# software-mansion/smelter

Measured on AMD Instinct MI355X. Metric: composited frames/sec, 8x1080p->1 4K scene, higher is better.
Workload: dtype u8 (f32 colour conversion: the WGSL sequence value for value; Lanczos on f16-pair MFMA with f32 accumulate, f16 resampler intermediate); 1 GPU; configs[2]: 8x1080p YUV420 inputs tiled -> 3840x2160 YUV420, Tiles + Rescaler(border_radius 24) + text label per tile, GpuOptimized (linear-light Lanczos3 + blend); inputs=8, layouts=33, prime_frames=4804, input_ring=12, frames_in_flight=2, parallelism=single GPU

## Files before the change

### smelter_amd/csrc/smr_fused_compose.h

```cpp
#pragma once

#include <type_traits>

#include "smr_convert_dev.h"
#include "smr_layout_dev.h"

namespace {

#ifdef SMR_EMU
#define B_KEEP_IN_LOOP(x) do { } while (0)
#else
#define B_KEEP_IN_LOOP(x) asm volatile("" : "+v"(x))
#endif

__device__ __forceinline__ u32 b_off(int row, u32 pitch, int col_bytes) { return (u32)__umul24((u32)row, pitch) + (u32)col_bytes; }

constexpr int B_TILE_W = 128, B_TILE_H = 16;
constexpr int B_MAX_LAYOUTS = 48;
constexpr int B_MAX_MASKS = 96;
static_assert(sizeof(DevLayout) % 16 == 0 && sizeof(DevMask) % 16 == 0, "LDS copies move 16 B words");

#ifndef SMR_COMPOSE_MIN_WAVES
#define SMR_COMPOSE_MIN_WAVES 6
#endif
constexpr int B_MIN_WAVES = SMR_COMPOSE_MIN_WAVES;
constexpr int B_BAND_ROWS = SMR_COMPOSE_BAND_ROWS;
static_assert(B_TILE_H % B_BAND_ROWS == 0 && B_BAND_ROWS >= 2, "a band fits the LDS pixel state");

inline u32 compose_predict(const PackedLayouts &p, int tiles_x, int tiles_y, std::vector<u32> &bitmap) {
    const int tiles = tiles_x * tiles_y, words = (tiles + 31) / 32;
    bitmap.assign((size_t)words, 0u);
    auto mark = [&](float x0, float y0, float x1, float y1) {
        int tx0 = (int)floorf(x0 / (float)B_TILE_W), tx1 = (int)floorf(x1 / (float)B_TILE_W);
        int ty0 = (int)floorf(y0 / (float)B_TILE_H), ty1 = (int)floorf(y1 / (float)B_TILE_H);
        tx0 = tx0 < 0 ? 0 : tx0; ty0 = ty0 < 0 ? 0 : ty0;
        tx1 = tx1 >= tiles_x ? tiles_x - 1 : tx1; ty1 = ty1 >= tiles_y ? tiles_y - 1 : ty1;
        for (int ty = ty0; ty <= ty1; ty++)
            for (int tx = tx0; tx <= tx1; tx++) {
                const int t = ty * tiles_x + tx;
                bitmap[t >> 5] |= 1u << (t & 31);
            }
    };
    auto corners = [&](float left, float top, float w, float h, float c, const DevLayout &L) {
        if (!(c > 0.0f)) return;
        const float bx0 = (float)L.bx0, by0 = (float)L.by0, bx1 = (float)L.bx1 - 1.0f, by1 = (float)L.by1 - 1.0f;
        const float xs[2][2] = {{left, left + c}, {left + w - c, left + w}}, ys[2][2] = {{top, top + c}, {top + h - c, top + h}};
        for (int a = 0; a < 2; a++)
            for (int b = 0; b < 2; b++) {
                const float x0 = fmaxf(xs[a][0], bx0), x1 = fminf(xs[a][1], bx1), y0 = fmaxf(ys[b][0], by0), y1 = fminf(ys[b][1], by1);
                if (x0 <= x1 && y0 <= y1) mark(x0, y0, x1, y1);
            }
    };
    for (int i = 0; i < p.n; i++) {
        const DevLayout &L = p.host_layouts[i];
        if (L.bx1 <= L.bx0 || L.by1 <= L.by0) continue;
        const bool solid_capable = (L.flags & DL_UNROTATED) && (L.type == 0 ? L.src_kind == 2 : (L.flags & DL_COLOR_OPAQUE) != 0);
        if (!solid_capable) {
            mark((float)L.bx0, (float)L.by0, (float)L.bx1 - 1.0f, (float)L.by1 - 1.0f);
            continue;
        }
        corners(L.left, L.top, L.width, L.height, L.corner, L);
        for (u32 m = 0; m < L.masks_len; m++) {
            const DevMask &K = p.host_masks[L.masks_off + m];
            corners(K.left, K.top, K.width, K.height, K.corner, L);
            if (K.left > L.left || K.top > L.top || K.left + K.width < L.left + L.width || K.top + K.height < L.top + L.height)
                mark((float)L.bx0, (float)L.by0, (float)L.bx1 - 1.0f, (float)L.by1 - 1.0f);
        }
        if (L.inset != 0.5f) {
            const float d = ceilf(L.inset);
            const float x0 = (float)L.bx0, y0 = (float)L.by0, x1 = (float)L.bx1 - 1.0f, y1 = (float)L.by1 - 1.0f;
            mark(x0, y0, x1, fminf(y0 + d, y1)); mark(x0, fmaxf(y1 - d, y0), x1, y1);
            mark(x0, y0, fminf(x0 + d, x1), y1); mark(fmaxf(x1 - d, x0), y0, x1, y1);
        }
    }
    u32 nf = 0;
    for (int w = 0; w < words; w++) nf += (u32)__builtin_popcount(bitmap[w]);
    return nf;
}

__device__ __forceinline__ void classify_layouts(u32 *s_touch, u32 *s_solid, int *s_start, const DevLayout *__restrict__ layouts,
                                                 const DevMask *__restrict__ masks, int n, int x0, int y0, int x1, int y1, int tid,
                                                 int nthreads) {
    if (tid < MAX_LAYOUT_WORDS) { s_touch[tid] = 0; s_solid[tid] = 0; }
    if (tid == 0) *s_start = -1;
    __syncthreads();
    const float cx0 = (float)x0 + 0.5f, cx1 = (float)x1 - 0.5f, cy0 = (float)y0 + 0.5f, cy1 = (float)y1 - 0.5f;
    for (int i = tid; i < n; i += nthreads) {
        const DevLayout &L = layouts[i];
        if (!(L.bx0 < x1 && L.bx1 > x0 && L.by0 < y1 && L.by1 > y0)) continue;
        atomicOr(&s_touch[i >> 5], 1u << (i & 31));
        if (!layout_solid_box(L, masks, cx0, cy0, cx1, cy1)) continue;
        atomicOr(&s_solid[i >> 5], 1u << (i & 31));
        if (layout_base_opaque(L)) atomicMax(s_start, i);
    }
    __syncthreads();
}

__device__ __forceinline__ void tile_needs(const u32 *s_touch, int start, int *s_general, const DevLayout *__restrict__ layouts, int n, int tid,
                                           int nthreads) {
    for (int i = tid; i < n; i += nthreads) {
        if (!((s_touch[i >> 5] >> (i & 31)) & 1u) || i < start) continue;
        const DevLayout &L = layouts[i];
        const bool copy_layer = i == start && (L.type != 0 || (L.flags & DL_ALIGNED));
        const bool sample_layer = i == start && L.type == 0 && !(L.flags & DL_ALIGNED);
        if (sample_layer) atomicOr(s_general, 2);
        else if (!copy_layer) atomicOr(s_general, 1);
        if (!(layout_base_opaque(L) && (L.flags & DL_UNROTATED))) atomicOr(s_general, 4);
    }
}

enum { TC_CLEAR = 0, TC_COLOUR = 1, TC_TEXTURE = 2, TC_FULL = 3, TC_SKIP = 4, TC_SAMPLED = 5, TC_SELECT = 6 };
struct alignas(16) TileClass {
    const u8 *base;
    u32 pitch_or_px;
    u32 kind;
};
struct TileFull {
    u32 tile;
    int start;
    u32 general;
    u32 band;
    u32 touch[MAX_LAYOUT_WORDS];
};
constexpr int B_AREA_BANDS = 4, B_EDGE_BANDS = B_TILE_H / B_BAND_ROWS;
static_assert(B_TILE_H / B_AREA_BANDS <= B_BAND_ROWS && B_EDGE_BANDS <= B_AREA_BANDS, "a band fits the workgroup's pixel state");
constexpr int B_LIST_COUNTERS = 64;
struct TileList {
    u32 count[B_LIST_COUNTERS];
    TileFull e[1];
};
constexpr u32 B_CLASS_NONE = 0xffu;
constexpr int B_CLASSIFY_TILES = 16;
__global__ __launch_bounds__(64 * B_CLASSIFY_TILES) void k_classify_tiles(const DevLayout *__restrict__ layouts, const DevMask *__restrict__ masks, int n,
                                                                          int W, int H, int tiles_x, int tiles, unsigned long long direct_layers,
                                                                          TileClass *__restrict__ tc, u8 *__restrict__ direct, TileList *__restrict__ full,
                                                                          int allow_select, int counter) {
    __shared__ u32 s_touch_w[B_CLASSIFY_TILES][MAX_LAYOUT_WORDS], s_solid_w[B_CLASSIFY_TILES][MAX_LAYOUT_WORDS];
    __shared__ int s_start_w[B_CLASSIFY_TILES], s_general_w[B_CLASSIFY_TILES], s_slot_w[B_CLASSIFY_TILES];
    __shared__ TileClass s_class_w[B_CLASSIFY_TILES];
    __shared__ u32 s_direct_w[B_CLASSIFY_TILES];
    const int wave = threadIdx.x >> 6, tid = threadIdx.x & 63;
    const bool live = (int)blockIdx.x * B_CLASSIFY_TILES + wave < tiles;
    const int tile = min((int)blockIdx.x * B_CLASSIFY_TILES + wave, tiles - 1);
    u32 *s_touch = s_touch_w[wave], *s_solid = s_solid_w[wave];
    int &s_start = s_start_w[wave], &s_general = s_general_w[wave], &s_slot = s_slot_w[wave];
    const int tile_y = tile / tiles_x;
    const int tx0 = (tile - tile_y * tiles_x) * B_TILE_W, ty0 = tile_y * B_TILE_H;
    if (tid == 0) s_general = 0;
    classify_layouts(s_touch, s_solid, &s_start, layouts, masks, n, tx0, ty0, min(tx0 + B_TILE_W, W), min(ty0 + B_TILE_H, H), tid, 64);
    const int start = s_start;
    tile_needs(s_touch, start, &s_general, layouts, n, tid, 64);
    __syncthreads();
    if (tid == 0) {
        TileClass c;
        c.base = nullptr; c.pitch_or_px = 0u; c.kind = TC_FULL;
        u32 d = B_CLASS_NONE;
        if ((s_general & 3) == 1 && allow_select) {
            const int x1 = min(tx0 + B_TILE_W, W), y1 = min(ty0 + B_TILE_H, H);
            u32 ids = 0xffffffffu;
            int cnt = 0;
            bool ok = true;
            for (int wi = (n + 31) / 32 - 1; ok && wi >= 0; wi--) {
                u32 bits = s_touch[wi];
                while (ok && bits) {
                    const int b = 31 - __clz(bits);
                    bits &= ~(1u << b);
                    const int i = wi * 32 + b;
                    if (i < start) continue;
                    const DevLayout &L = layouts[i];
                    const int ax0 = max(L.bx0, tx0), ay0 = max(L.by0, ty0), ax1 = min(L.bx1, x1), ay1 = min(L.by1, y1);
                    ok = cnt < 4 && i < 255 && layout_base_opaque(L) && (L.type != 0 || (L.flags & DL_ALIGNED)) &&
                         layout_solid_box(L, masks, (float)ax0 + 0.5f, (float)ay0 + 0.5f, (float)ax1 - 0.5f, (float)ay1 - 0.5f);
                    if (ok) {
                        ids = (ids & ~(0xffu << (8 * cnt))) | ((u32)i << (8 * cnt));
                        cnt++;
                    }
                }
            }
            if (ok && cnt > 0) {
                c.kind = TC_SELECT;
                c.pitch_or_px = ids;
            }
        } else if ((s_general & 3) == 2 && start >= 0) {
            c.kind = TC_SAMPLED;
            c.pitch_or_px = (u32)start;
        } else if ((s_general & 3) == 0) {
            if (start < 0) {
                c.kind = TC_CLEAR;
            } else if (layouts[start].type != 0) {
                c.kind = TC_COLOUR;
                c.pitch_or_px = layouts[start].solid_px;
            } else {
                const DevLayout &L = layouts[start];
                c.kind = TC_TEXTURE;
                c.base = L.src.ptr + (ptrdiff_t)(ty0 - L.iy) * (ptrdiff_t)L.src.pitch + (ptrdiff_t)(tx0 - L.ix) * 4;
                c.pitch_or_px = (u32)L.src.pitch;
                if (start < 64 && ((direct_layers >> start) & 1ull) && tx0 + B_TILE_W <= W && ty0 + B_TILE_H <= H) {
                    c.kind = TC_SKIP;
                    d = (u32)start;
                }
            }
        }
        s_slot = (live && c.kind == TC_FULL) ? ((s_general & 4) ? B_AREA_BANDS : B_EDGE_BANDS) : 0;
        s_class_w[wave] = c;
        s_direct_w[wave] = d;
    }
    __syncthreads();
    if (threadIdx.x == 0) {
        int want = 0;
        for (int w = 0; w < B_CLASSIFY_TILES; w++) want += s_slot_w[w];
        const u32 base = want ? atomicAdd(&full->count[counter], (u32)want) : 0u;
        int at = 0;
        for (int w = 0; w < B_CLASSIFY_TILES; w++) {
            const int mine = s_slot_w[w] ? (int)base + at : -1;
            at += s_slot_w[w];
            s_slot_w[w] = mine;
        }
    }
    __syncthreads();
    const int bands = (s_general & 4) ? B_AREA_BANDS : B_EDGE_BANDS;
    if (tid == 0 && live) {
        TileClass c = s_class_w[wave];
        if (c.kind == TC_FULL) { c.pitch_or_px = (u32)s_slot; c.base = (const u8 *)(uintptr_t)bands; }
        tc[tile] = c;
        direct[tile] = (u8)s_direct_w[wave];
    }
    if (s_slot >= 0) {
        const int rows = B_TILE_H / bands;
        for (int j = 0; j < bands; j++) {
            TileFull &E = full->e[s_slot + j];
            if (tid < MAX_LAYOUT_WORDS) E.touch[tid] = tid < ((n + 31) >> 5) ? s_touch[tid] : 0u;
            if (tid == 0) { E.tile = (u32)tile; E.start = start; E.general = (u32)s_general; E.band = (u32)(j * rows) | ((u32)rows << 8); }
        }
    }
}

template <typename T>
__device__ __forceinline__ T load_uniform(const T *p) {
    static_assert(sizeof(T) % 4 == 0, "dword records only");
    T out;
#pragma unroll
    for (int i = 0; i < (int)(sizeof(T) / 4); i++) {
        u32 w;
        __builtin_memcpy(&w, (const char *)p + 4 * i, 4);
        w = __builtin_amdgcn_readfirstlane(w);
        __builtin_memcpy((char *)&out + 4 * i, &w, 4);
    }
    return out;
}

__device__ __forceinline__ float4 decode_texel(u32 raw, int srgb, const float *__restrict__ dec) {
    const u32 r = raw & 0xff, g = (raw >> 8) & 0xff, b = (raw >> 16) & 0xff, a = raw >> 24;
    float4 o;
    if (srgb) { o.x = dec[r]; o.y = dec[g]; o.z = dec[b]; }
    else { o.x = (float)r / 255.0f; o.y = (float)g / 255.0f; o.z = (float)b / 255.0f; }
    o.w = div_cr((float)a, 255.0f, 1.0f / 255.0f);
    return o;
}

__device__ __forceinline__ u32 aligned_texel(const DevLayout &L, int px, int py) {
    return g_ld_u32(L.src.ptr + b_off(clampi(py - L.iy, 0, L.tex_h - 1), L.src.pitch, clampi(px - L.ix, 0, L.tex_w - 1) * 4));
}

__device__ __forceinline__ u32 compose_px(u32 a, const DevLayout &L, const DevMask *__restrict__ masks, int px, int py, bool is_base,
                                          u32 raw_pre, int srgb, const float *__restrict__ dec, const float *__restrict__ thr) {
    float fx, fy, lx, ly;
    if (!layout_covers(L, px, py, fx, fy, lx, ly)) return a;
    const bool solid = is_base || layout_solid_box(L, masks, fx, fy, fx, fy);
    if (L.type != 0) {
        if (solid && (L.flags & DL_COLOR_OPAQUE)) return L.solid_px;
        const float4 frag = solid ? make_float4(L.color[0], L.color[1], L.color[2], L.color[3])
                                  : layout_fragment(L, masks, fx, fy, lx, ly, make_float4(0.f, 0.f, 0.f, 0.f));
        return blend_store(a, frag, srgb, dec, thr);
    }
    const bool aligned = (L.flags & DL_ALIGNED) && L.src_kind != 0;
    u32 raw = 0u;
    float4 sample;
    if (aligned) {
        raw = raw_pre;
        sample = decode_texel(raw, srgb, dec);
    } else {
        sample = layout_texture_sample(L, px, py, lx, ly, srgb, dec);
    }
    const float4 frag = solid ? sample : layout_fragment(L, masks, fx, fy, lx, ly, sample);
    if (aligned && (raw >> 24) == 255u && frag.x == sample.x && frag.y == sample.y && frag.z == sample.z && frag.w == sample.w) return raw;
    return blend_store(a, frag, srgb, dec, thr);
}

__device__ __forceinline__ void yuv_block_repair(const u32 (&acc)[8], u32 &yrow0, u32 &yrow1, u32 &u2, u32 &v2) {
    u32 px[8];
    float r[8], g[8], b[8];
#pragma unroll
    for (int k = 0; k < 8; k++) {
        px[k] = acc[k];
        B_KEEP_IN_LOOP(px[k]);
        r[k] = unorm_of_byte(px[k] & 0xffu);
        g[k] = unorm_of_byte((px[k] >> 8) & 0xffu);
        b[k] = unorm_of_byte((px[k] >> 16) & 0xffu);
    }
#pragma unroll
    for (int k = 0; k < 8; k++) {
        bool f;
        (void)yuvfast::convert<0>((float)(px[k] & 0xffu), (float)((px[k] >> 8) & 0xffu), (float)((px[k] >> 16) & 0xffu), &f);
        const u32 exact = yuv_byte(r[k], g[k], b[k], 0), sh = 8u * (u32)(k & 3);
        u32 &row = k < 4 ? yrow0 : yrow1;
        row = f ? ((row & ~(0xffu << sh)) | (exact << sh)) : row;
    }
#pragma unroll
    for (int j = 0; j < 2; j++) {
        const int a = 2 * j, c = 4 + 2 * j;
        float sum[3];
#pragma unroll
        for (int ch = 0; ch < 3; ch++)
            sum[ch] = ((float)((px[a] >> (8 * ch)) & 0xffu) + (float)((px[a + 1] >> (8 * ch)) & 0xffu)) +
                      ((float)((px[c] >> (8 * ch)) & 0xffu) + (float)((px[c + 1] >> (8 * ch)) & 0xffu));
        bool f1, f2;
        (void)yuvfast::convert<1>(sum[0], sum[1], sum[2], &f1);
        (void)yuvfast::convert<2>(sum[0], sum[1], sum[2], &f2);
        const float mr = ((r[a] + r[a + 1]) + (r[c] + r[c + 1])) * 0.25f, mg = ((g[a] + g[a + 1]) + (g[c] + g[c + 1])) * 0.25f,
                    mb = ((b[a] + b[a + 1]) + (b[c] + b[c + 1])) * 0.25f;
        const u32 eu = yuv_byte(mr, mg, mb, 1), ev = yuv_byte(mr, mg, mb, 2), sh = 8u * (u32)j;
        u2 = f1 ? ((u2 & ~(0xffu << sh)) | (eu << sh)) : u2;
        v2 = f2 ? ((v2 & ~(0xffu << sh)) | (ev << sh)) : v2;
    }
}


__device__ __forceinline__ void yuv_block_repair_422(const u32 (&acc)[8], u32 &yrow0, u32 &yrow1, u32 &uv0, u32 &uv1) {
    u32 px[8];
    float r[8], g[8], b[8];
#pragma unroll
    for (int k = 0; k < 8; k++) {
        px[k] = acc[k];
        B_KEEP_IN_LOOP(px[k]);
        r[k] = unorm_of_byte(px[k] & 0xffu);
        g[k] = unorm_of_byte((px[k] >> 8) & 0xffu);
        b[k] = unorm_of_byte((px[k] >> 16) & 0xffu);
    }
#pragma unroll
    for (int k = 0; k < 8; k++) {
        bool f;
        (void)yuvfast::convert<0>((float)(px[k] & 0xffu), (float)((px[k] >> 8) & 0xffu), (float)((px[k] >> 16) & 0xffu), &f);
        const u32 exact = yuv_byte(r[k], g[k], b[k], 0), sh = 8u * (u32)(k & 3);
        u32 &row = k < 4 ? yrow0 : yrow1;
        row = f ? ((row & ~(0xffu << sh)) | (exact << sh)) : row;
    }
#pragma unroll
    for (int q = 0; q < 4; q++) {
        const int a = 4 * (q >> 1) + 2 * (q & 1);
        float sum[3];
#pragma unroll
        for (int ch = 0; ch < 3; ch++) sum[ch] = (float)((px[a] >> (8 * ch)) & 0xffu) + (float)((px[a + 1] >> (8 * ch)) & 0xffu);
        bool f1, f2;
        (void)yuvfast::convert422<1>(sum[0], sum[1], sum[2], &f1);
        (void)yuvfast::convert422<2>(sum[0], sum[1], sum[2], &f2);
        const float mr = r[a] * 0.5f + r[a + 1] * 0.5f, mg = g[a] * 0.5f + g[a + 1] * 0.5f, mb = b[a] * 0.5f + b[a + 1] * 0.5f;
        const u32 eu = yuv_byte(mr, mg, mb, 1), ev = yuv_byte(mr, mg, mb, 2), su = 8u * (u32)(q & 1), sv = su + 16u;
        u32 &uv = q < 2 ? uv0 : uv1;
        uv = f1 ? ((uv & ~(0xffu << su)) | (eu << su)) : uv;
        uv = f2 ? ((uv & ~(0xffu << sv)) | (ev << sv)) : uv;
    }
}

template <int NV>
__device__ __forceinline__ u32 packed422_texel(u32 y4, u32 uv, int j) {
    const u32 ya = (y4 >> (16 * j)) & 0xffu, yb = (y4 >> (16 * j + 8)) & 0xffu, u = (uv >> (8 * j)) & 0xffu, v = (uv >> (16 + 8 * j)) & 0xffu;
    return NV == 3 ? u | (ya << 8) | (v << 16) | (yb << 24) : ya | (u << 8) | (yb << 16) | (v << 24);
}

__device__ __forceinline__ bool plane_pair_aligned_422(const SurfView &p) { return ((((uintptr_t)p.ptr) | p.pitch) & 15u) == 0; }

template <int NV>
__device__ __forceinline__ void store_packed422_block(const u32 (&acc)[8], int px0, int py0, int W, const SurfView &p, bool pair) {
    float cr[8], cg[8], cb[8];
#pragma unroll
    for (int k = 0; k < 8; k++) {
        cr[k] = (float)(acc[k] & 0xffu);
        cg[k] = (float)((acc[k] >> 8) & 0xffu);
        cb[k] = (float)((acc[k] >> 16) & 0xffu);
    }
    u32 yrow0 = 0, yrow1 = 0, uv0 = 0, uv1 = 0;
    bool flagged = false;
#pragma unroll
    for (int k = 0; k < 4; k++) {
        bool f0, f1;
        yrow0 |= yuvfast::convert<0>(cr[k], cg[k], cb[k], &f0) << (8 * k);
        yrow1 |= yuvfast::convert<0>(cr[4 + k], cg[4 + k], cb[4 + k], &f1) << (8 * k);
        flagged |= f0 | f1;
    }
#pragma unroll
    for (int q = 0; q < 4; q++) {
        const int a = 4 * (q >> 1) + 2 * (q & 1);
        const float sr = cr[a] + cr[a + 1], sg = cg[a] + cg[a + 1], sb = cb[a] + cb[a + 1];
        bool f1, f2;
        const u32 c = (yuvfast::convert422<1>(sr, sg, sb, &f1) << (8 * (q & 1))) | (yuvfast::convert422<2>(sr, sg, sb, &f2) << (16 + 8 * (q & 1)));
        if (q < 2) uv0 |= c; else uv1 |= c;
        flagged |= f1 | f2;
    }
    if (flagged) {
        YUV_SLOW_PATH_STAYS_A_BRANCH();
        yuv_block_repair_422(acc, yrow0, yrow1, uv0, uv1);
    }
    const u32 t00 = packed422_texel<NV>(yrow0, uv0, 0), t01 = packed422_texel<NV>(yrow0, uv0, 1);
    const u32 t10 = packed422_texel<NV>(yrow1, uv1, 0), t11 = packed422_texel<NV>(yrow1, uv1, 1);
    if (pair) {
        const bool odd = (px0 & 4) != 0;
        const u32 n0 = (u32)dev_mov_dpp_quad_swap((int)(odd ? t00 : t10)), n1 = (u32)dev_mov_dpp_quad_swap((int)(odd ? t01 : t11));
        g_st_u32x4(p.ptr + b_off(py0 + (odd ? 1 : 0), p.pitch, (px0 & ~7) * 2), odd ? make_uint4(n0, n1, t10, t11) : make_uint4(t00, t01, n0, n1));
        return;
    }
    u8 *o = p.ptr + b_off(py0, p.pitch, px0 * 2);
    if (px0 + 3 >= W) {
        g_st_u32(o, t00);
        g_st_u32(o + p.pitch, t10);
    } else {
        g_st_u32x2(o, t00, t01);
        g_st_u32x2(o + p.pitch, t10, t11);
    }
}

template <int NV>
__device__ __forceinline__ bool planes_pair_aligned(const SurfView &yp, const SurfView &up, const SurfView &vp) {
#if defined(SMR_EMU) && !defined(SMR_EMU_WAVE_EXCHANGE)
    return false;
#else
    if (NV >= 3) return plane_pair_aligned_422(yp);
    if (NV == 2) return false;
    bool ok = ((((uintptr_t)yp.ptr) | yp.pitch) & 7u) == 0;
    if (NV == 0) ok = ok && ((((uintptr_t)up.ptr) | up.pitch | ((uintptr_t)vp.ptr) | vp.pitch) & 3u) == 0;
    return ok;
#endif
}

template <int NV>
__device__ __forceinline__ void store_yuv_block(const u32 (&acc)[8], int px0, int py0, int W, const SurfView &yp, const SurfView &up, const SurfView &vp,
                                                bool pair = false) {
    if (NV >= 3) {
        store_packed422_block<NV>(acc, px0, py0, W, yp, pair);
        return;
    }
    const bool half = px0 + 3 >= W;
    if (NV == 2) {
        u8 *o = yp.ptr + b_off(py0, yp.pitch, px0 * 4);
        if (half) {
            *(uint2 *)o = make_uint2(acc[0], acc[1]);
            *(uint2 *)(o + yp.pitch) = make_uint2(acc[4], acc[5]);
        } else {
            *(uint4 *)o = make_uint4(acc[0], acc[1], acc[2], acc[3]);
            *(uint4 *)(o + yp.pitch) = make_uint4(acc[4], acc[5], acc[6], acc[7]);
        }
        return;
    }
    float cr[8], cg[8], cb[8];
#pragma unroll
    for (int k = 0; k < 8; k++) {
        cr[k] = (float)(acc[k] & 0xffu);
        cg[k] = (float)((acc[k] >> 8) & 0xffu);
        cb[k] = (float)((acc[k] >> 16) & 0xffu);
    }
    u32 yrow0 = 0, yrow1 = 0, u2 = 0, v2 = 0;
    bool flagged = false;
#pragma unroll
    for (int k = 0; k < 4; k++) {
        bool f0, f1;
        yrow0 |= yuvfast::convert<0>(cr[k], cg[k], cb[k], &f0) << (8 * k);
        yrow1 |= yuvfast::convert<0>(cr[4 + k], cg[4 + k], cb[4 + k], &f1) << (8 * k);
        flagged |= f0 | f1;
    }
#pragma unroll
    for (int j = 0; j < 2; j++) {
        const int a = 2 * j, b = 2 * j + 1, c = 4 + 2 * j, d = 4 + 2 * j + 1;
        const float sr = (cr[a] + cr[b]) + (cr[c] + cr[d]), sg = (cg[a] + cg[b]) + (cg[c] + cg[d]), sb = (cb[a] + cb[b]) + (cb[c] + cb[d]);
        bool f1, f2;
        u2 |= yuvfast::convert<1>(sr, sg, sb, &f1) << (8 * j);
        v2 |= yuvfast::convert<2>(sr, sg, sb, &f2) << (8 * j);
        flagged |= f1 | f2;
    }
    if (flagged) {
        YUV_SLOW_PATH_STAYS_A_BRANCH();
        yuv_block_repair(acc, yrow0, yrow1, u2, v2);
    }
    const u32 uv4 = (u2 & 0xffu) | ((v2 & 0xffu) << 8) | ((u2 & 0xff00u) << 8) | ((v2 & 0xff00u) << 16);
    const int cx = px0 >> 1, cy = py0 >> 1;
    if (pair) {
        const bool odd = (px0 & 4) != 0;
        const u32 ny = (u32)dev_mov_dpp_quad_swap((int)(odd ? yrow0 : yrow1));
        g_st_u32x2(yp.ptr + b_off(py0 + (odd ? 1 : 0), yp.pitch, px0 & ~7), odd ? ny : yrow0, odd ? yrow1 : ny);
        if (NV == 0) {
            const u32 nc = (u32)dev_mov_dpp_quad_swap((int)(odd ? u2 : v2));
            u8 *o = odd ? vp.ptr + b_off(cy, vp.pitch, cx & ~3) : up.ptr + b_off(cy, up.pitch, cx);
            g_st_u32(o, odd ? (nc | (v2 << 16)) : (u2 | (nc << 16)));
        } else {
            *(u32 *)(up.ptr + b_off(cy, up.pitch, cx * 2)) = uv4;
        }
        return;
    }
    if (half) {
        *(u16 *)(yp.ptr + b_off(py0, yp.pitch, px0)) = (u16)yrow0;
        *(u16 *)(yp.ptr + b_off(py0 + 1, yp.pitch, px0)) = (u16)yrow1;
    } else {
        *(u32 *)(yp.ptr + b_off(py0, yp.pitch, px0)) = yrow0;
        *(u32 *)(yp.ptr + b_off(py0 + 1, yp.pitch, px0)) = yrow1;
    }
    if (NV == 0) {
        if (half) {
            up.ptr[b_off(cy, up.pitch, cx)] = (u8)u2;
            vp.ptr[b_off(cy, vp.pitch, cx)] = (u8)v2;
        } else {
            *(u16 *)(up.ptr + b_off(cy, up.pitch, cx)) = (u16)u2;
            *(u16 *)(vp.ptr + b_off(cy, vp.pitch, cx)) = (u16)v2;
        }
    } else if (half) {
        *(u16 *)(up.ptr + b_off(cy, up.pitch, cx * 2)) = (u16)uv4;
    } else {
        *(u32 *)(up.ptr + b_off(cy, up.pitch, cx * 2)) = uv4;
    }
}

__device__ __forceinline__ u32 list_slot(u32 *count, bool want) {
#ifdef SMR_EMU
    return want ? atomicAdd(count, 1u) : 0u;
#else
    const unsigned long long m = __ballot(want);
    if (m == 0ull) return 0u;
    const u32 rank = __builtin_amdgcn_mbcnt_hi((u32)(m >> 32), __builtin_amdgcn_mbcnt_lo((u32)m, 0u));
    u32 base = 0u;
    if (want && rank == 0u) base = atomicAdd(count, (u32)__popcll(m));
    return (u32)__builtin_amdgcn_readlane((int)base, (int)__builtin_ctzll(m)) + rank;
#endif
}
__device__ __forceinline__ bool wave_any(bool v) {
#ifdef SMR_EMU
    return true;
#else
    return __ballot(v) != 0ull;
#endif
}

template <int NV, bool BIG>
__device__ __forceinline__ void compose_full(const TileFull *__restrict__ pre, int band, int rh, const SurfView &yp, const SurfView &up, const SurfView &vp, int W, int H,
                                             const DevLayout *__restrict__ layouts_g, const DevMask *__restrict__ masks_g, int n, int n_masks,
                                             int srgb_and_ablate, const float *__restrict__ tables, int tiles_x, float *s_tab) {
    const int tile = (int)pre->tile;
    constexpr int BAND_PX = B_TILE_W * B_BAND_ROWS;
    constexpr int SWEEPS = 2;
    static_assert(BAND_PX % 512 == 0 && BAND_PX <= 2048, "whole slabs; a list entry keeps the pixel's index in IDX_BITS bits");
    constexpr int IDX_BITS = BIG ? 11 : (BAND_PX <= 1024 ? 10 : 11);
    constexpr bool WIDE = BIG || ((B_MAX_LAYOUTS + 1) > (1 << (16 - IDX_BITS)));
    typedef typename std::conditional<WIDE, u32, u16>::type entry_t;
    __shared__ u32 s_touch[MAX_LAYOUT_WORDS];
    __shared__ u32 s_px[BAND_PX];
    __shared__ entry_t s_list[BAND_PX];
    __shared__ u32 s_count;
    __shared__ __attribute__((aligned(16))) DevLayout s_lay[B_MAX_LAYOUTS];
    __shared__ __attribute__((aligned(16))) DevMask s_mask[B_MAX_MASKS];
    int tid = threadIdx.x;
    B_KEEP_IN_LOOP(tid);
    tid &= 255;
    u32 acc[8] = {0u, 0u, 0u, 0u, 0u, 0u, 0u, 0u};
    const int tile_y = tile / tiles_x;
    const int tx0 = (tile - tile_y * tiles_x) * B_TILE_W, ty0 = tile_y * B_TILE_H + band;
    const int px0 = tx0 + 4 * (tid & 31), py0 = ty0 + 2 * (tid >> 5);
    __syncthreads();
    {
        static_assert(SMR_TABLE_FLOATS % 4 == 0 && SMR_TABLE_FLOATS / 4 <= 256, "one 16 B word of the tables per thread");
        constexpr int LW = (B_MAX_LAYOUTS * (int)(sizeof(DevLayout) / 16) + 255) / 256, MW = (B_MAX_MASKS * (int)(sizeof(DevMask) / 16) + 255) / 256;
        const uint4 *gl = (const uint4 *)layouts_g, *gm = (const uint4 *)masks_g, *gt = (const uint4 *)tables;
        const int nl = BIG ? 0 : n * (int)(sizeof(DevLayout) / 16), nm = BIG ? 0 : n_masks * (int)(sizeof(DevMask) / 16);
        uint4 wl[LW], wm[MW], wt = make_uint4(0u, 0u, 0u, 0u);
#pragma unroll
        for (int k = 0; k < LW; k++) {
            wl[k] = wt;
            if (tid + 256 * k < nl) wl[k] = gl[tid + 256 * k];
        }
#pragma unroll
        for (int k = 0; k < MW; k++) {
            wm[k] = wt;
            if (tid + 256 * k < nm) wm[k] = gm[tid + 256 * k];
        }
        if (tid < SMR_TABLE_FLOATS / 4) wt = gt[tid];
        u32 touch_w = 0u;
        if (tid < MAX_LAYOUT_WORDS) touch_w = pre->touch[tid];
#pragma unroll
        for (int k = 0; k < LW; k++)
            if (tid + 256 * k < nl) ((uint4 *)s_lay)[tid + 256 * k] = wl[k];
#pragma unroll
        for (int k = 0; k < MW; k++)
            if (tid + 256 * k < nm) ((uint4 *)s_mask)[tid + 256 * k] = wm[k];
        if (tid < SMR_TABLE_FLOATS / 4) ((uint4 *)s_tab)[tid] = wt;
        if (tid < MAX_LAYOUT_WORDS) s_touch[tid] = touch_w;
        if (tid == 0) s_count = 0u;
    }
    const DevLayout *layouts = BIG ? layouts_g : s_lay;
    const DevMask *masks = BIG ? masks_g : s_mask;
    const int srgb = srgb_and_ablate & 1;
    const int ablate = srgb_and_ablate >> 8;
    const int start = pre->start;
    __syncthreads();
    if (ablate & (1 | 2 | 16)) return;
    if (ty0 >= H) return;
    const int words = (n + 31) >> 5;
    const bool no_block = px0 >= W || py0 >= H || 2 * (tid >> 5) >= rh;
    const int nsweeps = (B_TILE_W * rh) / 256;
    const float *dec = s_tab, *thr = s_tab + 256;
    const int sx = tx0 + (tid & (B_TILE_W - 1));

#pragma unroll 1
    for (int slab = 0; slab < nsweeps; slab += SWEEPS) {
    enum { K_NONE = 0, K_COLOUR = 1, K_TEXEL = 2, K_QUAD = 3 };
    int sp[SWEEPS];
    u32 kind[SWEEPS];
    const u8 *sbase[SWEEPS];
    u32 so[SWEEPS][4];
    float swx[SWEEPS], swy[SWEEPS];
#pragma unroll
    for (int s = 0; s < SWEEPS; s++) { sp[s] = -1; kind[s] = K_NONE; sbase[s] = nullptr; so[s][0] = so[s][1] = so[s][2] = so[s][3] = 0u; swx[s] = swy[s] = 0.0f; }
    const auto claim = [&](const DevLayout &L, int li, int s, int py) {
        sp[s] = li;
        if (L.type != 0) {
            kind[s] = K_COLOUR;
            so[s][0] = L.solid_px;
        } else if (L.flags & DL_ALIGNED) {
            kind[s] = K_TEXEL;
            sbase[s] = L.src.ptr;
            so[s][0] = (u32)b_off(clampi(py - L.iy, 0, L.tex_h - 1), L.src.pitch, clampi(sx - L.ix, 0, L.tex_w - 1) * 4);
        } else {
            kind[s] = K_QUAD;
            sbase[s] = L.src.ptr;
            const SampledAxis X = sampled_axis_x(L, sx), Y = sampled_axis_y(L, py);
            so[s][0] = Y.o0 + X.o0; so[s][1] = Y.o0 + X.o1; so[s][2] = Y.o1 + X.o0; so[s][3] = Y.o1 + X.o1;
            swx[s] = X.f; swy[s] = Y.f;
        }
    };
    for (int wi = (ablate & 4) ? -1 : words - 1; wi >= (start < 0 ? 0 : (start >> 5)); wi--) {
        u32 bits = __builtin_amdgcn_readfirstlane(s_touch[wi]);
        if (start >= 0 && wi == (start >> 5)) bits &= ~((2u << (start & 31)) - 1u);
        while (bits) {
            const int b = 31 - __builtin_clz(bits);
            bits &= ~(1u << b);
            const int li = (wi << 5) + b;
            const DevLayout L = load_uniform(&layouts[li]);
            if (!layout_base_opaque(L) || !(L.flags & DL_UNROTATED)) continue;
#pragma unroll
            for (int s = 0; s < SWEEPS; s++) {
                const int py = ty0 + (tid >> 7) + 2 * (slab + s);
                const float fx = (float)sx + 0.5f, fy = (float)py + 0.5f;
                if (slab + s < nsweeps && kind[s] == K_NONE && layout_solid_box(L, masks, fx, fy, fx, fy)) claim(L, li, s, py);
            }
        }
    }
    if (start >= 0) {
        const DevLayout L = load_uniform(&layouts[start]);
#pragma unroll
        for (int s = 0; s < SWEEPS; s++)
            if (slab + s < nsweeps && kind[s] == K_NONE) claim(L, start, s, ty0 + (tid >> 7) + 2 * (slab + s));
    }
    u32 st[SWEEPS][4];
#pragma unroll
    for (int s = 0; s < SWEEPS; s++) {
        st[s][0] = st[s][1] = st[s][2] = st[s][3] = 0u;
        if (kind[s] >= K_TEXEL) st[s][0] = g_ld_u32(sbase[s] + so[s][0]);
        if (kind[s] == K_QUAD) { st[s][1] = g_ld_u32(sbase[s] + so[s][1]); st[s][2] = g_ld_u32(sbase[s] + so[s][2]); st[s][3] = g_ld_u32(sbase[s] + so[s][3]); }
    }
    u32 val[SWEEPS];
#pragma unroll
    for (int s = 0; s < SWEEPS; s++) {
        val[s] = kind[s] == K_COLOUR ? so[s][0] : kind[s] == K_TEXEL ? st[s][0] : 0u;
        if (kind[s] == K_QUAD) val[s] = filter_opaque_quad(st[s][0], st[s][1], st[s][2], st[s][3], swx[s], swy[s], srgb, dec, thr);
    }

    bool listed[SWEEPS];
#pragma unroll
    for (int s = 0; s < SWEEPS; s++) listed[s] = false;
    if (!(ablate & 8))
        for (int wi = start < 0 ? 0 : (start >> 5); wi < words; wi++) {
            u32 bits = __builtin_amdgcn_readfirstlane(s_touch[wi]);
            if (start >= 0 && wi == (start >> 5)) bits &= ~((2u << (start & 31)) - 1u);
            while (bits) {
                const int li = (wi << 5) + __builtin_ctz(bits);
                bits &= bits - 1;
                const DevLayout *Lp = &layouts[li];
                const int bx0 = __builtin_amdgcn_readfirstlane(Lp->bx0), bx1 = __builtin_amdgcn_readfirstlane(Lp->bx1);
                const int by0 = __builtin_amdgcn_readfirstlane(Lp->by0), by1 = __builtin_amdgcn_readfirstlane(Lp->by1);
#pragma unroll
                for (int s = 0; s < SWEEPS; s++) {
                    const int py = ty0 + (tid >> 7) + 2 * (slab + s);
                    if (li > sp[s] && sx >= bx0 && sx < bx1 && py >= by0 && py < by1) listed[s] = true;
                }
            }
        }
#pragma unroll
    for (int s = 0; s < SWEEPS; s++) {
        if (slab + s >= nsweeps) break;
        const int idx = (slab + s) * 256 + tid, py = ty0 + (tid >> 7) + 2 * (slab + s);
        s_px[idx] = val[s];
        const bool want = listed[s] && sx < W && py < H;
        const u32 slot = list_slot(&s_count, want);
        if (want) s_list[slot] = (entry_t)((u32)idx | ((u32)(sp[s] + 1) << IDX_BITS));
    }
    }
    __syncthreads();

    const u32 total = s_count;
#pragma unroll 1
    for (u32 k0 = 0; k0 < total; k0 += 256u) {
        const bool act = k0 + (u32)tid < total;
        const u32 e = act ? (u32)s_list[k0 + tid] : 0u;
        const int idx = (int)(e & ((1u << IDX_BITS) - 1u)), from = (int)(e >> IDX_BITS) - 1;
        const int px = tx0 + (idx & (B_TILE_W - 1)), py = ty0 + (idx >> 7);
        u32 a = s_px[idx];
        for (int wi = start < 0 ? 0 : (start >> 5); wi < words; wi++) {
            u32 bits = __builtin_amdgcn_readfirstlane(s_touch[wi]);
            if (start >= 0 && wi == (start >> 5)) bits &= ~((2u << (start & 31)) - 1u);
            while (bits) {
                const int li = (wi << 5) + __builtin_ctz(bits);
                bits &= bits - 1;
                const DevLayout *Lp = &layouts[li];
                const int bx0 = __builtin_amdgcn_readfirstlane(Lp->bx0), bx1 = __builtin_amdgcn_readfirstlane(Lp->bx1);
                const int by0 = __builtin_amdgcn_readfirstlane(Lp->by0), by1 = __builtin_amdgcn_readfirstlane(Lp->by1);
                const bool need = act && li > from && px >= bx0 && px < bx1 && py >= by0 && py < by1;
                if (!wave_any(need)) continue;
                const DevLayout L = load_uniform(Lp);
                u32 raw = 0u;
                if (need && L.type == 0 && (L.flags & DL_ALIGNED) && L.src_kind != 0) raw = aligned_texel(L, px, py);
                if (need) a = compose_px(a, L, masks, px, py, false, raw, srgb, dec, thr);
            }
        }
        if (act) s_px[idx] = a;
    }
    __syncthreads();
    if (!no_block) {
        int ltid = tid;
        B_KEEP_IN_LOOP(ltid);
        const int lx0 = 4 * (ltid & 31), ly0 = 2 * (ltid >> 5), px0 = tx0 + lx0, py0 = ty0 + ly0;
        const uint4 t0 = *(const uint4 *)&s_px[ly0 * B_TILE_W + lx0], t1 = *(const uint4 *)&s_px[(ly0 + 1) * B_TILE_W + lx0];
        acc[0] = t0.x; acc[1] = t0.y; acc[2] = t0.z; acc[3] = t0.w;
        acc[4] = t1.x; acc[5] = t1.y; acc[6] = t1.z; acc[7] = t1.w;
        const bool pair = tx0 + B_TILE_W <= W && tile_y * B_TILE_H + B_TILE_H <= H && (rh & 3) == 0 && planes_pair_aligned<NV>(yp, up, vp);
        store_yuv_block<NV>(acc, px0, py0, W, yp, up, vp, pair);
    }
}

constexpr int B_COPY_TILES = 1;
#ifndef SMR_COPY_RUN
#define SMR_COPY_RUN 2
#endif
constexpr int B_COPY_RUN = SMR_COPY_RUN;
static_assert(B_COPY_RUN >= 1 && B_COPY_RUN <= 4, "a short run: the grid stays larger than what is resident");

__device__ __forceinline__ void copy_tile_texels(const TileClass &c, bool on, int cols, int bx, int by, const float *__restrict__ tables, u32 (&t)[8]) {
    const u32 fill = c.kind == TC_COLOUR ? c.pitch_or_px : 0u;
#pragma unroll
    for (int q = 0; q < 8; q++) t[q] = fill;
    if (c.kind != TC_TEXTURE) return;
    const bool aligned = ((((uintptr_t)c.base) | c.pitch_or_px) & 15) == 0 && !((cols & 3) != 0 && cols < B_TILE_W);
    if (aligned) {
        const u8 *r0 = on ? c.base + b_off(by, c.pitch_or_px, bx * 4) : (const u8 *)tables;
        const u8 *r1 = on ? r0 + c.pitch_or_px : (const u8 *)tables;
        const uint4 ra = g_ld_u32x4(r0), rb = g_ld_u32x4(r1);
        t[0] = ra.x; t[1] = ra.y; t[2] = ra.z; t[3] = ra.w;
        t[4] = rb.x; t[5] = rb.y; t[6] = rb.z; t[7] = rb.w;
    } else if (on) {
        const u8 *r0 = c.base + b_off(by, c.pitch_or_px, bx * 4), *r1 = r0 + c.pitch_or_px;
#pragma unroll
        for (int q = 0; q < 4; q++)
            if (bx + q < cols) { t[q] = g_ld_u32(r0 + 4 * q); t[4 + q] = g_ld_u32(r1 + 4 * q); }
    }
}

template <int NV, bool BIG>
__global__ __launch_bounds__(256, B_MIN_WAVES) void k_compose_output(SurfView yp, SurfView up, SurfView vp, int W, int H,
                                                        const DevLayout *__restrict__ layouts_g, const DevMask *__restrict__ masks_g,
                                                        int n, int n_masks, int srgb_and_ablate, const float *__restrict__ tables,
                                                        int tiles_x, int tiles, const TileClass *__restrict__ tc, const TileList *__restrict__ full,
                                                        int n_banded, int counter) {
    const int tid = threadIdx.x;
#if defined(SMR_PRIO_COMPOSE) && !defined(SMR_EMU)
    __builtin_amdgcn_s_setprio(SMR_PRIO_COMPOSE);
#endif
    __shared__ __attribute__((aligned(16))) float s_tab[SMR_TABLE_FLOATS];
    const int rest = (int)blockIdx.x - n_banded;
    int t_begin = 0, t_end = 0;
    bool later = false, left_out = false;
    if (rest < 0) {
        if (blockIdx.x >= full->count[counter]) return;
    } else {
        const int groups = (int)gridDim.x - n_banded;
        const int run = (tiles + groups - 1) / groups;
        t_begin = rest * run;
        t_end = min(t_begin + run, tiles);
        if (t_begin >= t_end) return;
        const bool ablate_copy = ((srgb_and_ablate >> 8) & 64) != 0;
        const bool planes_ok = planes_pair_aligned<NV>(yp, up, vp);
        int t = t_begin;
        const int ty = t / tiles_x;
        int tx0 = (t - ty * tiles_x) * B_TILE_W, ty0 = ty * B_TILE_H;
        TileClass c0 = tc[t], c1 = tc[min(t + 1, tiles - 1)], c2;
        u32 cur[8];
        copy_tile_texels(c0, tx0 + 4 * (tid & 31) < W && ty0 + 2 * (tid >> 5) < H && !ablate_copy, W - tx0, 4 * (tid & 31), 2 * (tid >> 5), tables, cur);
#pragma unroll 1
        for (;;) {
            int ltid = tid;
            B_KEEP_IN_LOOP(ltid);
            const int bx = 4 * (ltid & 31), by = 2 * (ltid >> 5);
            const int px0 = tx0 + bx, py0 = ty0 + by;
            const bool inside = px0 < W && py0 < H;
            const bool pair = planes_ok && tx0 + B_TILE_W <= W && ty0 + B_TILE_H <= H;
            c2 = tc[min(t + 2, tiles - 1)];
            u32 nxt[8] = {0u, 0u, 0u, 0u, 0u, 0u, 0u, 0u};
            const bool wrap = tx0 + B_TILE_W >= tiles_x * B_TILE_W;
            const int nx0 = wrap ? 0 : tx0 + B_TILE_W, ny0 = wrap ? ty0 + B_TILE_H : ty0;
            if (t + 1 < t_end) copy_tile_texels(c1, nx0 + bx < W && ny0 + by < H && !ablate_copy, W - nx0, bx, by, tables, nxt);
            if (c0.kind <= TC_TEXTURE) {
                if (inside && !ablate_copy) store_yuv_block<NV>(cur, px0, py0, W, yp, up, vp, pair);
            } else if (c0.kind == TC_SAMPLED || c0.kind == TC_SELECT) {
                later = true;
            } else if (c0.kind == TC_FULL && (int)c0.pitch_or_px + (int)(uintptr_t)c0.base > n_banded) {
                left_out = true;
            }
            if (++t >= t_end) break;
#pragma unroll
            for (int q = 0; q < 8; q++) cur[q] = nxt[q];
            c0 = c1; c1 = c2;
            tx0 = nx0; ty0 = ny0;
        }
        if (!later && !left_out) return;
    }
    if (later) {
#pragma unroll 1
        for (int t = t_begin; t < t_end; t++) {
            const TileClass c = tc[t];
            if (c.kind != TC_SAMPLED && c.kind != TC_SELECT) continue;
            int ltid = tid;
            B_KEEP_IN_LOOP(ltid);
            const int ty = t / tiles_x, tx0 = (t - ty * tiles_x) * B_TILE_W, ty0 = ty * B_TILE_H;
            const int px0 = tx0 + 4 * (ltid & 31), py0 = ty0 + 2 * (ltid >> 5);
            const bool inside = px0 < W && py0 < H;
            const bool pair = tx0 + B_TILE_W <= W && ty0 + B_TILE_H <= H && planes_pair_aligned<NV>(yp, up, vp);
            if (c.kind == TC_SAMPLED) {
                if ((srgb_and_ablate >> 8) & 32) continue;
                __syncthreads();
                for (int i = ltid; i < SMR_TABLE_FLOATS; i += 256) s_tab[i] = tables[i];
                __syncthreads();
                const DevLayout L = load_uniform(&layouts_g[c.pitch_or_px]);
                if (inside) {
                    u32 a[8];
                    composite_sampled_opaque_block(L, px0, py0, srgb_and_ablate & 1, s_tab, s_tab + 256, a);
                    store_yuv_block<NV>(a, px0, py0, W, yp, up, vp, pair);
                }
            } else if (c.kind == TC_SELECT) {
                u32 a[8] = {0u, 0u, 0u, 0u, 0u, 0u, 0u, 0u};
                u32 open_px = 0xffu;
#pragma unroll 1
                for (int q = 0; q < 4; q++) {
                    const u32 li = (c.pitch_or_px >> (8 * q)) & 0xffu;
                    if (li == 0xffu) break;
                    const DevLayout &L = layouts_g[li];
                    const int lx0 = L.bx0, ly0 = L.by0, lx1 = L.bx1, ly1 = L.by1;
                    const bool colour = L.type != 0;
                    const u32 solid = L.solid_px;
#pragma unroll
                    for (int i = 0; i < 8; i++) {
                        const int px = px0 + (i & 3), py = py0 + (i >> 2);
                        if (((open_px >> i) & 1u) && px >= lx0 && px < lx1 && py >= ly0 && py < ly1) {
                            a[i] = colour ? solid : aligned_texel(L, px, py);
                            open_px &= ~(1u << i);
                        }
                    }
                }
                if (inside) store_yuv_block<NV>(a, px0, py0, W, yp, up, vp, pair);
            }
        }
        if (!left_out) return;
    }
#pragma unroll 1
    for (int t = t_begin;; t++) {
        const TileFull *e;
        int entries = 1;
        if (rest < 0) {
            e = &full->e[blockIdx.x];
        } else {
            if (t >= t_end) break;
            const TileClass c = tc[t];
            if (!(c.kind == TC_FULL && (int)c.pitch_or_px + (int)(uintptr_t)c.base > n_banded)) continue;
            e = &full->e[c.pitch_or_px];
            entries = (int)(uintptr_t)c.base;
        }
#ifndef SMR_COMPOSE_NO_FULL
#pragma unroll 1
        for (int j = 0; j < entries; j++) {
            if (rest >= 0 && (int)(e - full->e) + j < n_banded) continue;
            const u32 bw = __builtin_amdgcn_readfirstlane(e[j].band);
            compose_full<NV, BIG>(&e[j], (int)(bw & 0xffu), (int)(bw >> 8), yp, up, vp, W, H, layouts_g, masks_g, n, n_masks, srgb_and_ablate, tables, tiles_x, s_tab);
        }
#endif
        if (rest < 0) break;
    }
}

}
```

Before: 21010 frames/s.

## Resolve opaque base per 4-pixel run with vector texel loads and batched list slots

Reworks the opaque-base pass of the full-tile compositor so each thread handles a horizontal run of four pixels instead of sweeping single pixels. A run is classified once per layer as solid colour, aligned texels (fetched with one 16-byte load), or split (falling back to per-pixel claims). The shading and list-append paths are batched: one atomic per wave covers all four pixels, and the results go to LDS with a single uint4 store. It also exposes the area-band count as a compile-time knob. The cost is more registers per thread and an extra bounding-box test per run, and split runs now carry four sets of per-pixel state.

```diff
diff --git a/smelter_amd/csrc/smr_fused_compose.h b/smelter_amd/csrc/smr_fused_compose.h
--- a/smelter_amd/csrc/smr_fused_compose.h
+++ b/smelter_amd/csrc/smr_fused_compose.h
@@ -122,7 +122,10 @@
     u32 band;
     u32 touch[MAX_LAYOUT_WORDS];
 };
-constexpr int B_AREA_BANDS = 4, B_EDGE_BANDS = B_TILE_H / B_BAND_ROWS;
+#ifndef SMR_COMPOSE_AREA_BANDS
+#define SMR_COMPOSE_AREA_BANDS 4
+#endif
+constexpr int B_AREA_BANDS = SMR_COMPOSE_AREA_BANDS, B_EDGE_BANDS = B_TILE_H / B_BAND_ROWS;
 static_assert(B_TILE_H / B_AREA_BANDS <= B_BAND_ROWS && B_EDGE_BANDS <= B_AREA_BANDS, "a band fits the workgroup's pixel state");
 constexpr int B_LIST_COUNTERS = 64;
 struct TileList {
@@ -517,16 +520,28 @@
     }
 }
 
-__device__ __forceinline__ u32 list_slot(u32 *count, bool want) {
+__device__ __forceinline__ void list_slots4(u32 *count, u32 want4, u32 (&slot)[4]) {
 #ifdef SMR_EMU
-    return want ? atomicAdd(count, 1u) : 0u;
+#pragma unroll
+    for (int j = 0; j < 4; j++) slot[j] = ((want4 >> j) & 1u) ? atomicAdd(count, 1u) : 0u;
 #else
-    const unsigned long long m = __ballot(want);
-    if (m == 0ull) return 0u;
-    const u32 rank = __builtin_amdgcn_mbcnt_hi((u32)(m >> 32), __builtin_amdgcn_mbcnt_lo((u32)m, 0u));
+    unsigned long long m[4];
+    u32 first[4], total = 0u;
+#pragma unroll
+    for (int j = 0; j < 4; j++) {
+        m[j] = __ballot(((want4 >> j) & 1u) != 0u);
+        first[j] = total;
+        total += (u32)__popcll(m[j]);
+    }
+#pragma unroll
+    for (int j = 0; j < 4; j++) slot[j] = 0u;
+    if (total == 0u) return;
+    const u32 lane = __builtin_amdgcn_mbcnt_hi(~0u, __builtin_amdgcn_mbcnt_lo(~0u, 0u));
     u32 base = 0u;
-    if (want && rank == 0u) base = atomicAdd(count, (u32)__popcll(m));
-    return (u32)__builtin_amdgcn_readlane((int)base, (int)__builtin_ctzll(m)) + rank;
+    if (lane == 0u) base = atomicAdd(count, total);
+    base = (u32)__builtin_amdgcn_readlane((int)base, 0);
+#pragma unroll
+    for (int j = 0; j < 4; j++) slot[j] = base + first[j] + __builtin_amdgcn_mbcnt_hi((u32)(m[j] >> 32), __builtin_amdgcn_mbcnt_lo((u32)m[j], 0u));
 #endif
 }
 __device__ __forceinline__ bool wave_any(bool v) {
@@ -537,14 +552,67 @@
 #endif
 }
 
+enum { K_NONE = 0, K_COLOUR = 1, K_TEXEL = 2, K_QUAD = 3 };
+enum { R_OPEN = 0, R_COLOUR = 1, R_TEXELS = 2, R_SPLIT = 3 };
+struct RunPx {
+    int sp;
+    u32 kind;
+    const u8 *base;
+    u32 so, sdy, sw;
+    u32 t0, t1, t2, t3;
+};
+__device__ __forceinline__ void run_claim_px(RunPx &q, const DevLayout &L, const DevMask *__restrict__ masks, int li, int sx, int ry, bool everywhere) {
+    const float fx = (float)sx + 0.5f, fy = (float)ry + 0.5f;
+    if (q.kind != K_NONE || !(everywhere || layout_solid_box(L, masks, fx, fy, fx, fy))) return;
+    u32 kind, so, sdy = 0u, sw = 0u;
+    if (L.type != 0) {
+        kind = K_COLOUR;
+        so = L.solid_px;
+    } else if (L.flags & DL_ALIGNED) {
+        kind = K_TEXEL;
+        so = (u32)b_off(clampi(ry - L.iy, 0, L.tex_h - 1), L.src.pitch, clampi(sx - L.ix, 0, L.tex_w - 1) * 4);
+    } else {
+        kind = K_QUAD;
+        const SampledAxis X = sampled_axis_x(L, sx), Y = sampled_axis_y(L, ry);
+        so = Y.o0 + X.o0;
+        sdy = Y.o1 - Y.o0;
+        sw = (u32)(X.f * 256.0f) | ((u32)(Y.f * 256.0f) << 16) | (X.o1 != X.o0 ? 0x80000000u : 0u);
+    }
+    q.sp = li; q.kind = kind; q.base = L.src.ptr; q.so = so; q.sdy = sdy; q.sw = sw;
+}
+__device__ __forceinline__ void run_visit(int &run, RunPx &q0, RunPx &q1, RunPx &q2, RunPx &q3, const DevLayout &L, const DevMask *__restrict__ masks, int li,
+                                          int rx, int ry, bool everywhere) {
+    const float fx0 = (float)rx + 0.5f, fx3 = (float)rx + 3.5f, fy = (float)ry + 0.5f;
+    if (run == R_OPEN) {
+        if (everywhere || layout_solid_box(L, masks, fx0, fy, fx3, fy)) {
+            const int tx = rx - L.ix;
+            const u32 off = (u32)b_off(clampi(ry - L.iy, 0, L.tex_h - 1), L.src.pitch, tx * 4);
+            const bool texels = L.type == 0 && (L.flags & DL_ALIGNED) && tx >= 0 && tx + 3 < L.tex_w && (((uintptr_t)L.src.ptr + off) & 15u) == 0;
+            run = L.type != 0 ? R_COLOUR : texels ? R_TEXELS : R_SPLIT;
+            if (run != R_SPLIT) {
+                q0.sp = q1.sp = q2.sp = q3.sp = li;
+                q0.base = L.src.ptr;
+                q0.so = L.type != 0 ? L.solid_px : off;
+            }
+        } else if (!(fx3 < L.left + L.inset || fx0 > L.left + L.width - L.inset || fy < L.top + L.inset || fy > L.top + L.height - L.inset)) {
+            run = R_SPLIT;
+        }
+    }
+    if (run != R_SPLIT) return;
+    run_claim_px(q0, L, masks, li, rx, ry, everywhere);
+    run_claim_px(q1, L, masks, li, rx + 1, ry, everywhere);
+    run_claim_px(q2, L, masks, li, rx + 2, ry, everywhere);
+    run_claim_px(q3, L, masks, li, rx + 3, ry, everywhere);
+}
+
 template <int NV, bool BIG>
 __device__ __forceinline__ void compose_full(const TileFull *__restrict__ pre, int band, int rh, const SurfView &yp, const SurfView &up, const SurfView &vp, int W, int H,
                                              const DevLayout *__restrict__ layouts_g, const DevMask *__restrict__ masks_g, int n, int n_masks,
                                              int srgb_and_ablate, const float *__restrict__ tables, int tiles_x, float *s_tab) {
     const int tile = (int)pre->tile;
     constexpr int BAND_PX = B_TILE_W * B_BAND_ROWS;
-    constexpr int SWEEPS = 2;
-    static_assert(BAND_PX % 512 == 0 && BAND_PX <= 2048, "whole slabs; a list entry keeps the pixel's index in IDX_BITS bits");
+    constexpr int PASSES = B_BAND_ROWS > 8 ? B_BAND_ROWS / 8 : 1;
+    static_assert(BAND_PX % 512 == 0 && BAND_PX <= 2048 && B_BAND_ROWS % 8 == 0, "whole passes; a list entry keeps the pixel's index in IDX_BITS bits");
     constexpr int IDX_BITS = BIG ? 11 : (BAND_PX <= 1024 ? 10 : 11);
     constexpr bool WIDE = BIG || ((B_MAX_LAYOUTS + 1) > (1 << (16 - IDX_BITS)));
     typedef typename std::conditional<WIDE, u32, u16>::type entry_t;
@@ -601,37 +669,16 @@
     if (ty0 >= H) return;
     const int words = (n + 31) >> 5;
     const bool no_block = px0 >= W || py0 >= H || 2 * (tid >> 5) >= rh;
-    const int nsweeps = (B_TILE_W * rh) / 256;
     const float *dec = s_tab, *thr = s_tab + 256;
-    const int sx = tx0 + (tid & (B_TILE_W - 1));
-
 #pragma unroll 1
-    for (int slab = 0; slab < nsweeps; slab += SWEEPS) {
-    enum { K_NONE = 0, K_COLOUR = 1, K_TEXEL = 2, K_QUAD = 3 };
-    int sp[SWEEPS];
-    u32 kind[SWEEPS];
-    const u8 *sbase[SWEEPS];
-    u32 so[SWEEPS][4];
-    float swx[SWEEPS], swy[SWEEPS];
-#pragma unroll
-    for (int s = 0; s < SWEEPS; s++) { sp[s] = -1; kind[s] = K_NONE; sbase[s] = nullptr; so[s][0] = so[s][1] = so[s][2] = so[s][3] = 0u; swx[s] = swy[s] = 0.0f; }
-    const auto claim = [&](const DevLayout &L, int li, int s, int py) {
-        sp[s] = li;
-        if (L.type != 0) {
-            kind[s] = K_COLOUR;
-            so[s][0] = L.solid_px;
-        } else if (L.flags & DL_ALIGNED) {
-            kind[s] = K_TEXEL;
-            sbase[s] = L.src.ptr;
-            so[s][0] = (u32)b_off(clampi(py - L.iy, 0, L.tex_h - 1), L.src.pitch, clampi(sx - L.ix, 0, L.tex_w - 1) * 4);
-        } else {
-            kind[s] = K_QUAD;
-            sbase[s] = L.src.ptr;
-            const SampledAxis X = sampled_axis_x(L, sx), Y = sampled_axis_y(L, py);
-            so[s][0] = Y.o0 + X.o0; so[s][1] = Y.o0 + X.o1; so[s][2] = Y.o1 + X.o0; so[s][3] = Y.o1 + X.o1;
-            swx[s] = X.f; swy[s] = Y.f;
-        }
-    };
+    for (int pass = 0; pass < PASSES; pass++) {
+    const int rrow = 8 * pass + (tid >> 5), rpx = 4 * (256 * pass + tid);
+    const int rx = tx0 + 4 * (tid & 31), ry = ty0 + rrow;
+    const bool in_band = rrow < rh;
+
+    int run = in_band ? R_OPEN : R_COLOUR;
+    RunPx q0 = {-1, K_NONE, nullptr, 0u, 0u, 0u, 0u, 0u, 0u, 0u}, q1 = q0, q2 = q0, q3 = q0;
+#define B_EACH_PX(F) do { F(q0, 0); F(q1, 1); F(q2, 2); F(q3, 3); } while (0)
     for (int wi = (ablate & 4) ? -1 : words - 1; wi >= (start < 0 ? 0 : (start >> 5)); wi--) {
         u32 bits = __builtin_amdgcn_readfirstlane(s_touch[wi]);
         if (start >= 0 && wi == (start >> 5)) bits &= ~((2u << (start & 31)) - 1u);
@@ -641,37 +688,25 @@
             const int li = (wi << 5) + b;
             const DevLayout L = load_uniform(&layouts[li]);
             if (!layout_base_opaque(L) || !(L.flags & DL_UNROTATED)) continue;
-#pragma unroll
-            for (int s = 0; s < SWEEPS; s++) {
-                const int py = ty0 + (tid >> 7) + 2 * (slab + s);
-                const float fx = (float)sx + 0.5f, fy = (float)py + 0.5f;
-                if (slab + s < nsweeps && kind[s] == K_NONE && layout_solid_box(L, masks, fx, fy, fx, fy)) claim(L, li, s, py);
-            }
+            run_visit(run, q0, q1, q2, q3, L, masks, li, rx, ry, false);
         }
     }
     if (start >= 0) {
         const DevLayout L = load_uniform(&layouts[start]);
-#pragma unroll
-        for (int s = 0; s < SWEEPS; s++)
-            if (slab + s < nsweeps && kind[s] == K_NONE) claim(L, start, s, ty0 + (tid >> 7) + 2 * (slab + s));
-    }
-    u32 st[SWEEPS][4];
-#pragma unroll
-    for (int s = 0; s < SWEEPS; s++) {
-        st[s][0] = st[s][1] = st[s][2] = st[s][3] = 0u;
-        if (kind[s] >= K_TEXEL) st[s][0] = g_ld_u32(sbase[s] + so[s][0]);
-        if (kind[s] == K_QUAD) { st[s][1] = g_ld_u32(sbase[s] + so[s][1]); st[s][2] = g_ld_u32(sbase[s] + so[s][2]); st[s][3] = g_ld_u32(sbase[s] + so[s][3]); }
-    }
-    u32 val[SWEEPS];
-#pragma unroll
-    for (int s = 0; s < SWEEPS; s++) {
-        val[s] = kind[s] == K_COLOUR ? so[s][0] : kind[s] == K_TEXEL ? st[s][0] : 0u;
-        if (kind[s] == K_QUAD) val[s] = filter_opaque_quad(st[s][0], st[s][1], st[s][2], st[s][3], swx[s], swy[s], srgb, dec, thr);
-    }
-
-    bool listed[SWEEPS];
-#pragma unroll
-    for (int s = 0; s < SWEEPS; s++) listed[s] = false;
+        run_visit(run, q0, q1, q2, q3, L, masks, start, rx, ry, true);
+    }
+    uint4 wv = make_uint4(0u, 0u, 0u, 0u);
+    if (run == R_TEXELS) wv = g_ld_u32x4(q0.base + q0.so);
+    const auto fetch = [&](RunPx &q, int) __attribute__((always_inline)) {
+        if (q.kind >= K_TEXEL) q.t0 = g_ld_u32(q.base + q.so);
+        if (q.kind == K_QUAD) {
+            const u32 dx = (q.sw >> 31) * 4u;
+            q.t1 = g_ld_u32(q.base + (q.so + dx)); q.t2 = g_ld_u32(q.base + (q.so + q.sdy)); q.t3 = g_ld_u32(q.base + (q.so + q.sdy + dx));
+        }
+    };
+    if (run == R_SPLIT) B_EACH_PX(fetch);
+
+    u32 listed = 0u;
     if (!(ablate & 8))
         for (int wi = start < 0 ? 0 : (start >> 5); wi < words; wi++) {
             u32 bits = __builtin_amdgcn_readfirstlane(s_touch[wi]);
@@ -682,22 +717,33 @@
                 const DevLayout *Lp = &layouts[li];
                 const int bx0 = __builtin_amdgcn_readfirstlane(Lp->bx0), bx1 = __builtin_amdgcn_readfirstlane(Lp->bx1);
                 const int by0 = __builtin_amdgcn_readfirstlane(Lp->by0), by1 = __builtin_amdgcn_readfirstlane(Lp->by1);
-#pragma unroll
-                for (int s = 0; s < SWEEPS; s++) {
-                    const int py = ty0 + (tid >> 7) + 2 * (slab + s);
-                    if (li > sp[s] && sx >= bx0 && sx < bx1 && py >= by0 && py < by1) listed[s] = true;
-                }
+                if (!(in_band && ry >= by0 && ry < by1 && rx + 3 >= bx0 && rx < bx1)) continue;
+                const auto touch = [&](RunPx &q, int j) __attribute__((always_inline)) {
+                    if (li > q.sp && rx + j >= bx0 && rx + j < bx1) listed |= 1u << j;
+                };
+                B_EACH_PX(touch);
             }
         }
-#pragma unroll
-    for (int s = 0; s < SWEEPS; s++) {
-        if (slab + s >= nsweeps) break;
-        const int idx = (slab + s) * 256 + tid, py = ty0 + (tid >> 7) + 2 * (slab + s);
-        s_px[idx] = val[s];
-        const bool want = listed[s] && sx < W && py < H;
-        const u32 slot = list_slot(&s_count, want);
-        if (want) s_list[slot] = (entry_t)((u32)idx | ((u32)(sp[s] + 1) << IDX_BITS));
-    }
+    {
+        const auto value = [&](RunPx &q, int) __attribute__((always_inline)) {
+            if (q.kind == K_COLOUR) q.t0 = q.so;
+            if (q.kind == K_QUAD)
+                q.t0 = filter_opaque_quad(q.t0, q.t1, q.t2, q.t3, (float)(q.sw & 0xffffu) * (1.0f / 256.0f), (float)((q.sw >> 16) & 0x7fffu) * (1.0f / 256.0f), srgb, dec, thr);
+        };
+        B_EACH_PX(value);
+        if (run == R_COLOUR) wv = make_uint4(q0.so, q0.so, q0.so, q0.so);
+        if (run == R_SPLIT) wv = make_uint4(q0.t0, q1.t0, q2.t0, q3.t0);
+        if (in_band) *(uint4 *)&s_px[rpx] = wv;
+    }
+    if (ry >= H) listed = 0u;
+    if (rx + 3 >= W) listed &= (1u << (W > rx ? W - rx : 0)) - 1u;
+    u32 slot[4];
+    list_slots4(&s_count, listed, slot);
+    const auto enlist = [&](RunPx &q, int j) __attribute__((always_inline)) {
+        if ((listed >> j) & 1u) s_list[slot[j]] = (entry_t)((u32)(rpx + j) | ((u32)(q.sp + 1) << IDX_BITS));
+    };
+    B_EACH_PX(enlist);
+#undef B_EACH_PX
     }
     __syncthreads();
 
```

After: 20830 frames/s. About the same (-0.8%).
